# petuum/poseidon

Measured on AMD Instinct MI355X. Metric: images/sec (whole node), higher is better.
Workload: dtype bf16; 1 GPU; model=alexnet, global_batch=256, input=3x227x227, parallelism=dp1, sfb=False, hipgraph=True

## Files before the change

poseidon_amd/ops/csrc/bindings.cpp:

```cpp

#include <torch/extension.h>
#include <c10/hip/HIPStream.h>
#include <hip/hip_runtime.h>

#include <algorithm>
#include <atomic>
#include <cmath>
#include <cstdlib>
#include <utility>

#include "ps_api.h"
#include "ps_mt.h"

namespace {

using at::Tensor;

hipStream_t stream() { return c10::hip::getCurrentHIPStream().stream(); }

bool is_bf16(const Tensor& t) { return t.scalar_type() == at::kBFloat16; }

struct P {
  void* p;
  explicit P(const Tensor& t) : p(t.data_ptr()) {}
// ... 197 lines not shown
    const c10::optional<Tensor>& dw_acc,
    const c10::optional<Tensor>& dw_out) {
  check_float_like(dy, "dy");
  TORCH_CHECK(!(dw_acc.has_value() && dw_out.has_value()),
              "linear_backward: dw_acc and dw_out exclude each other");
  auto xc = x.contiguous();
  auto wc = linear_weight(w, w_shadow, is_bf16(dy));
  auto dyc = dy.contiguous();
  int M = xc.size(0), K = xc.size(1), N = wc.size(0);
  c10::optional<Tensor> dx, dw, db;
  if (need_dx) {
    Tensor t = at::empty({M, K}, x.options());
    run_gemm(dyc, wc, t, nullptr, M, K, N, N, K, K, 0, 0, 0, true, false,
             1.0f, 0.0f);
    dx = t;
  }
  if (need_dw) {
    const bool own = !dw_acc.has_value() && !dw_out.has_value();
    Tensor t = dw_acc.has_value() ? *dw_acc
               : dw_out.has_value()
                   ? *dw_out
                   : at::empty({N, K}, x.options().dtype(at::kFloat));
    TORCH_CHECK(t.is_cuda() && t.scalar_type() == at::kFloat &&
                t.is_contiguous() && t.dim() == 2 && t.size(0) == N &&
                t.size(1) == K,
                "linear_backward: dW target must be contiguous f32 [N,K]");
    run_gemm(dyc, xc, t, nullptr, N, K, M, N, K, K, 0, 0, 0, false, false,
             1.0f, dw_acc.has_value() ? 1.0f : 0.0f);
    if (own) dw = t;
  }
  if (has_bias) {
    Tensor t = at::zeros({N}, x.options().dtype(at::kFloat));
    colsum_into(dyc, t.data_ptr<float>(), M, N);
    db = t;
  }
  return {dx, dw, db};
}

Tensor gemm_at_b(const Tensor& a, const Tensor& b) {
  check_float_like(a, "a");
  auto ac = a.contiguous();
  auto bc = b.contiguous();
  int M = ac.size(0), N = ac.size(1), K = bc.size(1);
  Tensor t = at::empty({N, K}, a.options().dtype(at::kFloat));
  run_gemm(ac, bc, t, nullptr, N, K, M, N, K, K, 0, 0, 0, false, false,
           1.0f, 0.0f);
  return t;
}


enum { PS_PACKED_OFF = 0, PS_PACKED_ON = 1, PS_PACKED_AUTO = -1 };
enum { PS_ROWFUSED_OFF = 0, PS_ROWFUSED_ON = 1, PS_ROWFUSED_AUTO = -1 };

ConvPlan conv_plan_for(at::IntArrayRef x_shape, int Co, int kh, int kw,
                       int sh, int sw, int ph, int pw, int G, bool bf16,
                       int packed = PS_PACKED_AUTO,
                       int rowfused = PS_ROWFUSED_AUTO) {
  TORCH_CHECK(x_shape.size() == 4 && G > 0 && x_shape[1] % G == 0 &&
              Co % G == 0, "conv channel/group mismatch");
  const bool rf_auto = rowfused == PS_ROWFUSED_AUTO;
  const ConvPolicy policy = {
      g_implicit_gemm.load(), g_implicit_thresh.load(),
      g_dgrad_fwd_thresh.load(),
      packed == PS_PACKED_AUTO ? g_packed_conv.load() : packed == PS_PACKED_ON,
      rf_auto ? g_rowfused_conv.load() : rowfused == PS_ROWFUSED_ON,
      rf_auto ? g_rowfused_thresh.load() : 0,
      rf_auto && ps_deterministic() != 0};
  ConvPlan p = ps_conv_plan((int)x_shape[0], (int)x_shape[1], (int)x_shape[2],
                            (int)x_shape[3], Co, kh, kw, sh, sw, ph, pw, G,
                            bf16 ? 2 : 4, policy);
  if (p.rowfused && !ps_rowfused_prepare()) p.rowfused = false;
  return p;
}

py::dict conv_plan(std::vector<int64_t> x_shape, std::vector<int64_t> w_shape,
                   std::vector<int64_t> stride, std::vector<int64_t> pad,
                   int G, bool bf16) {
  TORCH_CHECK(w_shape.size() == 4 && stride.size() == 2 && pad.size() == 2);
  TORCH_CHECK(x_shape.size() == 4 && w_shape[1] * G == x_shape[1],
              "conv channel/group mismatch");
  const ConvPlan p = conv_plan_for(x_shape, (int)w_shape[0], (int)w_shape[2],
                                   (int)w_shape[3], (int)stride[0],
                                   (int)stride[1], (int)pad[0], (int)pad[1],
                                   G, bf16);
  py::dict d;
  d["N"] = p.g.N; d["C"] = p.g.C; d["H"] = p.g.H; d["W"] = p.g.W;
  d["Ho"] = p.g.Ho; d["Wo"] = p.g.Wo; d["G"] = p.g.G;
  d["Co"] = p.Co; d["Cg"] = p.Cg; d["Cog"] = p.Cog;
  d["Kg"] = p.Kg; d["Kcol"] = p.Kcol; d["NP"] = p.NP; d["vec"] = p.vec;
  d["is_1x1"] = p.is_1x1; d["ld_col"] = p.ld_col; d["wk_ld"] = p.wk_ld;
  d["kpad"] = p.kpad; d["implicit"] = p.implicit;
  d["Kgw_implicit"] = p.Kgw_implicit; d["dgrad_as_fwd"] = p.dgrad_as_fwd;
  d["packed"] = p.packed; d["pk_W"] = p.pk_W; d["pk_kw"] = p.pk_kw;
  d["pk_Kg"] = p.pk_Kg; d["kw_ld"] = p.kw_ld; d["c_ld"] = p.c_ld;
  d["rowfused"] = p.rowfused;
  d["Kgw"] = p.implicit ? p.Kgw_implicit : p.wk_ld;
  return d;
}

std::vector<int64_t> khwc_layout(int64_t Cg, int64_t kw, bool packed) {
  int kw_ld, c_ld;
  ps_khwc_layout((int)kw, (int)Cg, packed, &kw_ld, &c_ld);
  return {kw_ld, c_ld};
}

Tensor weight_khwc_tr(const Tensor& w, int G, bool bf16) {
// ... 10 lines not shown
std::vector<Tensor> conv2d_forward_ex(const Tensor& x, const Tensor& w,
                                      const c10::optional<Tensor>& bias,
                                      int sh, int sw, int ph, int pw, int G,
                                      bool fuse_relu,
                                      const c10::optional<Tensor>& wk_cached,
                                      const c10::optional<Tensor>& wkT_cached) {
  check_float_like(x, "x");
  const bool bf16 = is_bf16(x);
  TORCH_CHECK(x.dim() == 4 && w.size(1) * G == x.size(1),
              "conv channel/group mismatch");
  const ConvPlan p = conv_plan_for(x.sizes(), (int)w.size(0),
                                   (int)w.size(2), (int)w.size(3), sh, sw, ph,
                                   pw, G, bf16);
  const ConvGeom& g = p.g;
  const int Co = p.Co, Cog = p.Cog;
  Tensor x_cl = (p.is_1x1 || p.implicit) ? cl4(x) : Tensor();

  const auto cdt = bf16 ? at::kBFloat16 : at::kFloat;
  Tensor wk, wkT;
  if (wk_cached.has_value() && wkT_cached.has_value() &&
      wk_cached->scalar_type() == cdt) {
    TORCH_CHECK(wk_cached->size(1) == p.wk_ld, "conv2d_forward: cached wk is ",
                wk_cached->size(1), " wide, the plan's wk_ld is ", p.wk_ld);
    wk = *wk_cached;
    wkT = *wkT_cached;
  } else {
    auto wc = w.contiguous();
    auto wkopts = w.options().dtype(cdt);
    wk = p.kpad ? at::zeros({Co, (int64_t)p.wk_ld}, wkopts)
                : at::empty({Co, (int64_t)p.wk_ld}, wkopts);
    wkT = at::empty({(int64_t)p.Kcol, (int64_t)Cog}, wkopts);
    PS_CALL_W(weight_to_khwc_both, bf16, wc.data_ptr<float>(), P(wk), P(wkT),
            Co, p.Cg, g.kh, g.kw, G, p.wk_ld, p.kw_ld, p.c_ld, stream());
  }

  Tensor colT;
  if (p.rowfused) {
    TORCH_CHECK(x.numel() / g.N < (1LL << 31) &&
                (g.H - 1) * x.stride(2) + (g.W - 1) * x.stride(3) +
                (g.C - 1) * x.stride(1) < (1LL << 31),
                "row-fused conv: one image must span < 2^31 elements");
    TORCH_CHECK(wk.is_contiguous() && ((uintptr_t)wk.data_ptr() & 15) == 0,
                "row-fused conv: wk must be contiguous and 16 B aligned");
    const RowFusedTiling t = ps_rowfused_tiling(
        g.N, g.C, g.H, g.W, Co, g.kh, g.kw, g.sh, g.sw, g.ph, g.pw, p.wk_ld);
    Tensor y = empty_cl({g.N, Co, g.Ho, g.Wo}, x.options());
    Tensor bc;
    const float* bp = nullptr;
    if (bias.has_value()) {
      bc = bias->contiguous();
      bp = bc.data_ptr<float>();
    }
    ps_conv_rowfused_fwd(&t, x.data_ptr(), x.stride(0), x.stride(1),
                         x.stride(2), x.stride(3), wk.data_ptr(), bp,
                         y.data_ptr(), fuse_relu ? 1 : 0, stream());
    return {y, at::empty({0, (int64_t)p.ld_col}, x.options()), wkT};
  }
  if (p.packed) {
    colT = at::empty({g.N, g.H, (int64_t)p.pk_W, PS_PK_C}, x.options());
    ps_pack_pairs_bf16(x.data_ptr(), colT.data_ptr(), g.N, g.C, g.H, g.W,
                       p.pk_W, g.pw, x.stride(0), x.stride(1), x.stride(2),
                       x.stride(3), stream());
  } else if (p.is_1x1) {
    colT = rows2d(x_cl);
  } else if (!p.implicit) {
    colT = at::empty({p.NP, (int64_t)p.ld_col}, x.options());
    const bool staged = PS_CALL(im2col_rowstage, bf16, P(x), P(colT), &g,
                                p.ld_col, x.stride(0), x.stride(1),
                                x.stride(2), x.stride(3), stream());
    if (!staged) {
      const Tensor xc = cl4(x);
      PS_CALL(im2col_nhwc, bf16, P(xc), P(colT), &g, p.ld_col, stream());
      if (p.kpad)
        PS_CALL(zero_cols, bf16, P(colT), p.NP, p.ld_col, p.Kcol, stream());
    }
  }

  Tensor y = empty_cl({g.N, Co, g.Ho, g.Wo}, x.options());
  const float* bp = nullptr;
  Tensor bc;
  if (bias.has_value()) {
    bc = bias->contiguous();
    bp = bc.data_ptr<float>();
  }
  const int Kgl = p.wk_ld;
  const bool gather = p.implicit || p.packed;
  const Tensor& xg = p.packed ? colT : x_cl;
  for (int grp = 0; grp < G; ++grp) {
    GatherDesc ga{};
    if (gather)
      ga = ps_gather_desc(p, PS_GATHER_FWD, xg.data_ptr(), zero_page(xg), grp);
    run_gemm(gather ? xg : colT, wk, y, bp ? bp + grp * Cog : nullptr,
             (int)p.NP, Cog, Kgl,
             gather ? Kgl : p.ld_col, Kgl, Co,
             gather ? 0 : (int64_t)grp * Kgl,
             (int64_t)grp * Cog * Kgl,
             (int64_t)grp * Cog,
             true, true, 1.0f, 0.0f, gather ? &ga : nullptr, nullptr,
             fuse_relu);
  }
  if (!colT.defined())
    colT = at::empty({0}, x.options());
  return {y, colT, wkT};
}

Tensor conv2d_backward_input(const Tensor& w, const Tensor& dy,
                             std::vector<int64_t> x_shape, int sh, int sw,
                             int ph, int pw, int G,
// ... 38 lines not shown
  Tensor dcolT = p.is_1x1 ? rows2d(dx)
                          : at::empty({p.NP, (int64_t)p.Kcol}, dy.options());
  Tensor dy2 = rows2d(dy_cl);
  for (int grp = 0; grp < G; ++grp) {
    run_gemm(dy2, wkT, dcolT, nullptr,
             (int)p.NP, Kg, Cog,
             Co, Cog, p.Kcol,
             (int64_t)grp * Cog, (int64_t)grp * Kg * Cog,
             (int64_t)grp * Kg,
             true, true, 1.0f, 0.0f);
  }
  if (!p.is_1x1)
    PS_CALL(col2im_nhwc, bf16, P(dcolT), P(dx), &g, stream());
  return dx;
}

Tensor conv2d_backward_weight_acc(const Tensor& x, const Tensor& colT,
                                  const Tensor& dy, Tensor dw_out,
                                  c10::optional<Tensor> db_out,
                                  int sh, int sw, int ph, int pw, int G,
                                  const c10::optional<Tensor>& dwk_buf,
                                  bool skip_unpack, bool skip_db) {
  check_float_like(dy, "dy");
  auto dy_cl = cl4(dy);
  const bool implicit = colT.numel() == 0 && colT.dim() == 1;
  const bool packed = colT.dim() == 4;
  const bool rowfused = colT.dim() == 2 && colT.size(0) == 0;
  const ConvPlan p = conv_plan_for(x.sizes(), (int)dw_out.size(0),
                                   (int)dw_out.size(2), (int)dw_out.size(3),
                                   sh, sw, ph, pw, G, is_bf16(dy),
                                   packed ? PS_PACKED_ON : PS_PACKED_OFF,
                                   rowfused ? PS_ROWFUSED_ON : PS_ROWFUSED_OFF);
  TORCH_CHECK(dw_out.size(1) == p.Cg && dy_cl.size(2) == p.g.Ho &&
              dy_cl.size(3) == p.g.Wo, "conv wgrad: shape mismatch");
  const int Co = p.Co, Cog = p.Cog;
  if (rowfused) {
    TORCH_CHECK(p.rowfused && is_bf16(x) && is_bf16(dy),
                "conv wgrad: row-fused cache slot does not match the plan");
    TORCH_CHECK(!ps_deterministic(),
                "conv wgrad: the row-fused wgrad has no deterministic form");
    const ConvGeom& g = p.g;
    TORCH_CHECK(x.numel() / g.N < (1LL << 31) &&
                (g.H - 1) * x.stride(2) + (g.W - 1) * x.stride(3) +
                (g.C - 1) * x.stride(1) < (1LL << 31),
                "row-fused conv: one image must span < 2^31 elements");
    const int Kgw = p.wk_ld;
    const bool prez =
        dwk_buf.has_value() && dwk_buf->numel() == (int64_t)Co * Kgw;
    Tensor dwk = prez ? *dwk_buf
               : at::empty({Co, (int64_t)Kgw}, dy.options().dtype(at::kFloat));
    const RowFusedTiling t = ps_rowfused_tiling(
        g.N, g.C, g.H, g.W, Co, g.kh, g.kw, g.sh, g.sw, g.ph, g.pw, p.wk_ld);
    ps_conv_rowfused_wgrad(&t, x.data_ptr(), x.stride(0), x.stride(1),
                           x.stride(2), x.stride(3), dy_cl.data_ptr(),
                           dwk.data_ptr<float>(), prez ? 1 : 0, stream());
    if (!skip_unpack)
      ps_weight_from_khwc_f32(dwk.data_ptr<float>(), dw_out.data_ptr<float>(),
                              Co, p.Cg, g.kh, g.kw, Kgw,
                              1.0f, p.kw_ld, p.c_ld, stream());
    if (db_out.has_value() && !skip_db)
      colsum_into(dy_cl, db_out->data_ptr<float>(), p.NP, Co);
    return dwk;
  }
  if (packed) {
    TORCH_CHECK(p.packed && colT.is_contiguous() && is_bf16(colT) &&
                colT.size(0) == p.g.N && colT.size(1) == p.g.H &&
                colT.size(2) == p.pk_W && colT.size(3) == PS_PK_C,
                "conv wgrad: packed input does not match the plan");
  } else {
    TORCH_CHECK(implicit || colT.size(1) == p.ld_col,
                "conv wgrad: colT width does not match the plan");
  }
  const Tensor xg = packed ? colT : implicit ? cl4(x) : Tensor();
  const bool gather = implicit || packed;
  const int Kgw = implicit ? p.Kgw_implicit : p.wk_ld;

  const bool prez = dwk_buf.has_value() && dwk_buf->numel() == (int64_t)Co * Kgw;
  Tensor dwk = prez ? *dwk_buf
             : at::empty({Co, (int64_t)Kgw}, dy.options().dtype(at::kFloat));
  Tensor dy2 = rows2d(dy_cl);
  for (int grp = 0; grp < G; ++grp) {
    GatherDesc gb{};
    if (gather)
      gb = ps_gather_desc(p, PS_GATHER_WGRAD, xg.data_ptr(), zero_page(xg),
                          grp);
    run_gemm(dy2, gather ? xg : colT, dwk, nullptr,
             Cog, Kgw, (int)p.NP,
             Co, gather ? Kgw : p.ld_col, Kgw,
             (int64_t)grp * Cog,
             gather ? 0 : (int64_t)grp * Kgw,
             (int64_t)grp * Cog * Kgw,
             false, false, 1.0f, 0.0f, nullptr, gather ? &gb : nullptr,
             false, prez);
  }
  if (!skip_unpack)
    ps_weight_from_khwc_f32(dwk.data_ptr<float>(), dw_out.data_ptr<float>(),
                            Co, p.Cg, p.g.kh, p.g.kw, Kgw,
                            1.0f, p.kw_ld, p.c_ld, stream());
  if (db_out.has_value() && !skip_db)
    colsum_into(dy_cl, db_out->data_ptr<float>(), p.NP, Co);
  return dwk;
}


Tensor concat_channels(std::vector<Tensor> inputs) {
  TORCH_CHECK(!inputs.empty());
  auto x0 = cl4(inputs[0]);
  int64_t N = x0.size(0), H = x0.size(2), W = x0.size(3);
// ... 1025 lines not shown
```

poseidon_amd/ops/csrc/conv_rowfused.hip:

```cpp

#include "ps_common.h"
#include "ps_api.h"
#include "ps_rowfused.h"

#include <atomic>
#include <mutex>

namespace ps {
namespace {

constexpr int RF_THREADS = PS_RF_THREADS;
constexpr int RF_STAGERS = 256;

typedef __attribute__((ext_vector_type(4))) __bf16 rf_bf16x4;
typedef __attribute__((ext_vector_type(4))) int rf_i32x4;

struct RfX {
  const __bf16* x;
  int64_t sn;
  int sc, sh, sw;
};

__device__ inline __bf16 rf_read(const char* img, int pbase, int koff) {
  return *reinterpret_cast<const __bf16*>(img + max(pbase + koff, 0));
}

typedef __bf16 rf_uvec8 __attribute__((ext_vector_type(8), aligned(2)));

template <int NV, int NT>
__device__ inline void rf_load_x(bf16x8 (&xv)[NV], const RowFusedTiling& t,
                                 const RowFusedTile& tl, const RfX& X,
                                 int tid, int first) {
  const int vpr = t.rsw_ld / 8;
  const int total = t.srows * t.C * vpr;
  const int iw0 = tl.ow0 * t.sw - t.pw;
  const int ih0 = tl.oh0 * t.sh - t.ph;
  const __bf16* xn = X.x + tl.n * X.sn;
#pragma unroll
  for (int v = 0; v < NV; ++v) {
    const int idx = first + tid + v * NT;
    const int rc = idx / vpr;
    const int sr = rc / t.C;
    const int c = rc - sr * t.C;
    const int ih = ih0 + sr;
    const int iw = iw0 + (idx - rc * vpr) * 8;
#pragma unroll
    for (int j = 0; j < 8; ++j) xv[v][j] = (__bf16)0.0f;
    if (idx < total && ih >= 0 && ih < t.H) {
      const __bf16* src = xn + (ih * X.sh + c * X.sc);
      if (X.sw == 1 && iw >= 0 && iw + 8 <= t.W) {
        xv[v] = *reinterpret_cast<const rf_uvec8*>(src + iw);
      } else {
#pragma unroll
        for (int j = 0; j < 8; ++j)
          if (iw + j >= 0 && iw + j < t.W) xv[v][j] = src[(iw + j) * X.sw];
      }
    }
  }
}

template <int NV, int NT>
__device__ inline void rf_store_x(char* img, const bf16x8 (&xv)[NV],
                                  const RowFusedTiling& t, int tid,
                                  int first) {
  const int total = t.srows * t.C * (t.rsw_ld / 8);
#pragma unroll
  for (int v = 0; v < NV; ++v) {
    const int idx = first + tid + v * NT;
    if (idx < total)
      *reinterpret_cast<bf16x8*>(img + PS_RF_HDR + idx * 16) = xv[v];
  }
}

constexpr int RF_FV = 6;
__device__ inline void rf_stage_x(char* img, const RowFusedTiling& t,
                                  const RowFusedTile& tl, const RfX& X,
                                  int ptid) {
  const int total = t.srows * t.C * (t.rsw_ld / 8);
  for (int first = 0; first < total; first += RF_FV * RF_STAGERS) {
    bf16x8 xv[RF_FV];
    rf_load_x<RF_FV, RF_STAGERS>(xv, t, tl, X, ptid, first);
    rf_store_x<RF_FV, RF_STAGERS>(img, xv, t, ptid, first);
  }
}

__device__ inline void rf_zero_headers(char* xs0, int xs_bytes, int tid) {
  if (tid < 4) reinterpret_cast<int*>(xs0)[tid] = 0;
  else if (tid < 8) reinterpret_cast<int*>(xs0 + xs_bytes)[tid - 4] = 0;
}

template <int FN>
__global__ __launch_bounds__(RF_THREADS)
void conv_rowfused_fwd_k(RowFusedTiling t, RfX X,
                         const __bf16* __restrict__ wk,
                         const float* __restrict__ bias,
                         __bf16* __restrict__ y, int relu, float alpha,
                         int tpb) {
  extern __shared__ __attribute__((aligned(16))) char smem[];
  __bf16* wl = reinterpret_cast<__bf16*>(smem);
  int* kofft = reinterpret_cast<int*>(smem + t.fwd_koff_off);
  char* xs0 = smem + t.fwd_xs_off;
  const int tid = threadIdx.x;
  const int lane = tid & 63;
  const int wid = __builtin_amdgcn_readfirstlane(tid >> 6);
  const int l = lane & 15, q = lane >> 4;
  const int64_t t0 = (int64_t)blockIdx.x * tpb;
  const int64_t t1 = t0 + tpb < t.tiles ? t0 + tpb : t.tiles;
  if (t0 >= t1) return;

  {
    const int vpr = t.Kpad / 8;
    for (int i = tid; i < t.Cop * vpr; i += RF_THREADS) {
      const int co = i / vpr;
      const int kv = (i - co * vpr) * 8;
      bf16x8 v;
#pragma unroll
      for (int j = 0; j < 8; ++j) v[j] = (__bf16)0.0f;
      if (co < t.Co)
        v = *reinterpret_cast<const bf16x8*>(&wk[(int64_t)co * t.Kpad + kv]);
      *reinterpret_cast<bf16x8*>(&wl[co * t.w_ld + kv]) = v;
    }
    for (int k = tid; k < t.Kpad; k += RF_THREADS) kofft[k] = ps_rf_koff(t, k);
    rf_zero_headers(xs0, t.xs_bytes, tid);
  }
  if (wid >= 4)
    rf_stage_x(xs0, t, ps_rf_tile(t, t0), X, tid - RF_STAGERS);
  int pf[2], pbf[2];
#pragma unroll
  for (int f = 0; f < 2; ++f) {
    pf[f] = (wid & 3) * 32 + f * 16 + l;
    pbf[f] = ps_rf_pbase(t, pf[f]);
  }
  __syncthreads();

  for (int64_t ti = t0; ti < t1; ++ti) {
    const int cur = (int)(ti - t0) & 1;
    if (wid >= 4) {
      if (ti + 1 < t1)
        rf_stage_x(xs0 + (cur ^ 1) * t.xs_bytes, t, ps_rf_tile(t, ti + 1), X,
                   tid - RF_STAGERS);
    } else {
      const RowFusedTile tl = ps_rf_tile(t, ti);
      if (wid * 32 < tl.nlive) {
        const char* img = xs0 + cur * t.xs_bytes;
        int pb[2];
#pragma unroll
        for (int f = 0; f < 2; ++f)
          pb[f] = pf[f] < tl.nlive ? pbf[f] : PS_RF_NEG;
        f32x4 acc[2][FN] = {};
#pragma unroll 2
        for (int ks = 0; ks < t.Kpad; ks += 32) {
          const rf_i32x4 k0 =
              *reinterpret_cast<const rf_i32x4*>(&kofft[ks + q * 8]);
          const rf_i32x4 k1 =
              *reinterpret_cast<const rf_i32x4*>(&kofft[ks + q * 8 + 4]);
          bf16x8 bfr[FN];
#pragma unroll
          for (int fn = 0; fn < FN; ++fn)
            bfr[fn] = *reinterpret_cast<const bf16x8*>(
                &wl[(fn * 16 + l) * t.w_ld + ks + q * 8]);
          bf16x8 af[2];
#pragma unroll
          for (int f = 0; f < 2; ++f) {
#pragma unroll
            for (int e = 0; e < 4; ++e) {
              af[f][e] = rf_read(img, pb[f], k0[e]);
              af[f][4 + e] = rf_read(img, pb[f], k1[e]);
            }
          }
#pragma unroll
          for (int f = 0; f < 2; ++f)
#pragma unroll
            for (int fn = 0; fn < FN; ++fn)
              acc[f][fn] = __builtin_amdgcn_mfma_f32_16x16x32_bf16(
                  af[f], bfr[fn], acc[f][fn], 0, 0, 0);
        }
#pragma unroll
        for (int f = 0; f < 2; ++f) {
#pragma unroll
          for (int fn = 0; fn < FN; ++fn) {
            const int col = fn * 16 + l;
            if (col >= t.Co) continue;
            const float bv = bias ? bias[col] : 0.0f;
#pragma unroll
            for (int r = 0; r < 4; ++r) {
              const int p = wid * 32 + f * 16 + q * 4 + r;
              if (p >= tl.nlive) continue;
              float v = alpha * acc[f][fn][r] + bv;
              if (relu && v < 0.0f) v = 0.0f;
              from_f32(v, y[(tl.pos0 + p) * t.Co + col]);
            }
          }
        }
      }
    }
    __syncthreads();
  }
}

__device__ inline bf16x8 rf_tr_frag(unsigned base, int kk, int cb, int l,
                                    int ld) {
  const unsigned a1 =
      base + (unsigned)(((kk + (l >> 2)) * ld + cb + 4 * (l & 3)) * 2);
  const unsigned a2 = a1 + (unsigned)(4 * ld * 2);
  rf_bf16x4 v1, v2;
  asm volatile("ds_read_b64_tr_b16 %0, %2\n\t"
               "ds_read_b64_tr_b16 %1, %3"
               : "=&v"(v1), "=&v"(v2) : "v"(a1), "v"(a2));
  bf16x8 f;
#pragma unroll
  for (int i = 0; i < 4; ++i) { f[i] = v1[i]; f[4 + i] = v2[i]; }
  return f;
}

template <int N>
__device__ inline void rf_tr_wait(bf16x8 (&a)[N]) {
  asm volatile("s_waitcnt lgkmcnt(0)" ::: "memory");
#pragma unroll
  for (int i = 0; i < N; ++i) asm volatile("" : "+v"(a[i]));
}

template <int FN, int KF>
__global__ __launch_bounds__(RF_THREADS)
void conv_rowfused_wgrad_k(RowFusedTiling t, RfX X,
                           const __bf16* __restrict__ dy,
                           float* __restrict__ dwk, int tpb) {
  extern __shared__ __attribute__((aligned(16))) char smem[];
  int* ptab = reinterpret_cast<int*>(smem);
  __bf16* dyl0 = reinterpret_cast<__bf16*>(smem + t.wg_dy_off);
  char* xs0 = smem + t.wg_xs_off;
  const int dy_tile = PS_RF_TM * t.dy_ld;
  const int tid = threadIdx.x;
  const int lane = tid & 63;
  const int wid = __builtin_amdgcn_readfirstlane(tid >> 6);
  const int l = lane & 15, q = lane >> 4;
  const int64_t t0 = (int64_t)blockIdx.x * tpb;
  const int64_t t1 = t0 + tpb < t.tiles ? t0 + tpb : t.tiles;
  if (t0 >= t1) return;
  rf_zero_headers(xs0, t.xs_bytes, tid);

  const int my_pb = tid < PS_RF_TM ? ps_rf_pbase(t, tid) : 0;
  const int cv8 = t.Cop / 8;
  bf16x8 xv[PS_RF_XV], dv[PS_RF_DV];
  auto load = [&](int64_t ti) {
    const RowFusedTile tl = ps_rf_tile(t, ti);
    rf_load_x<PS_RF_XV, RF_THREADS>(xv, t, tl, X, tid, 0);
#pragma unroll
    for (int v = 0; v < PS_RF_DV; ++v) {
      const int idx = tid + v * RF_THREADS;
      const int p = idx / cv8;
      const int cv = (idx - p * cv8) * 8;
#pragma unroll
      for (int j = 0; j < 8; ++j) dv[v][j] = (__bf16)0.0f;
      if (p < tl.nlive && cv < t.Co)
        dv[v] = *reinterpret_cast<const bf16x8*>(
            &dy[(tl.pos0 + p) * t.Co + cv]);
    }
  };
  auto store = [&](int buf, int64_t ti) {
    const RowFusedTile tl = ps_rf_tile(t, ti);
    rf_store_x<PS_RF_XV, RF_THREADS>(xs0 + buf * t.xs_bytes, xv, t, tid,
                                     0);
    __bf16* dyl = dyl0 + buf * dy_tile;
#pragma unroll
    for (int v = 0; v < PS_RF_DV; ++v) {
      const int idx = tid + v * RF_THREADS;
      const int p = idx / cv8;
      const int cv = (idx - p * cv8) * 8;
      if (p < PS_RF_TM)
        *reinterpret_cast<bf16x8*>(&dyl[p * t.dy_ld + cv]) = dv[v];
    }
    if (tid < PS_RF_TM)
      ptab[buf * PS_RF_TM + tid] = tid < tl.nlive ? my_pb : PS_RF_NEG;
  };
  load(t0);
  store(0, t0);

  const int by = blockIdx.y;
  int kofs[KF];
  bool klive[KF];
#pragma unroll
  for (int i = 0; i < KF; ++i) {
    const int kf = (by * KF + i) * 8 + wid;
    klive[i] = kf * 16 < t.Kpad;
    kofs[i] = klive[i] ? ps_rf_koff(t, kf * 16 + l) : PS_RF_NEG;
  }
  f32x4 acc[FN][KF] = {};
  __syncthreads();

  for (int64_t ti = t0; ti < t1; ++ti) {
    const int cur = (int)(ti - t0) & 1;
    if (ti + 1 < t1) load(ti + 1);
    {
      const RowFusedTile tl = ps_rf_tile(t, ti);
      const char* img = xs0 + cur * t.xs_bytes;
      const int* pt = ptab + cur * PS_RF_TM;
      const unsigned dyb = (unsigned)(unsigned long long)(
          __attribute__((address_space(3))) __bf16*)(dyl0 + cur * dy_tile);
      for (int p0 = 0; p0 < tl.nlive; p0 += 32) {
        const rf_i32x4 pa =
            *reinterpret_cast<const rf_i32x4*>(&pt[p0 + q * 8]);
        const rf_i32x4 pb =
            *reinterpret_cast<const rf_i32x4*>(&pt[p0 + q * 8 + 4]);
        bf16x8 af[FN];
#pragma unroll
        for (int fn = 0; fn < FN; ++fn)
          af[fn] = rf_tr_frag(dyb, p0 + q * 8, fn * 16, l, t.dy_ld);
        rf_tr_wait(af);
#pragma unroll
        for (int i = 0; i < KF; ++i) {
          if (klive[i]) {
            bf16x8 bfr;
#pragma unroll
            for (int e = 0; e < 4; ++e) {
              bfr[e] = rf_read(img, pa[e], kofs[i]);
              bfr[4 + e] = rf_read(img, pb[e], kofs[i]);
            }
#pragma unroll
            for (int fn = 0; fn < FN; ++fn)
              acc[fn][i] = __builtin_amdgcn_mfma_f32_16x16x32_bf16(
                  af[fn], bfr, acc[fn][i], 0, 0, 0);
// ... 48 lines not shown
template <int FN>
void rf_launch_fwd(const RowFusedTiling& t, const RfX& X, const void* wk,
                   const float* bias, void* y, int relu, hipStream_t s) {
  int blocks, tpb;
  rf_grid(t, &blocks, &tpb);
  conv_rowfused_fwd_k<FN><<<dim3((unsigned)blocks), RF_THREADS, t.fwd_lds,
                            s>>>(t, X, (const __bf16*)wk, bias, (__bf16*)y,
                                 relu, 1.0f, tpb);
}

template <int FN, int KF>
void rf_launch_wgrad(const RowFusedTiling& t, const RfX& X, const void* dy,
                     float* dwk, hipStream_t s) {
  int blocks, tpb;
  rf_grid(t, &blocks, &tpb);
  const int gy = (t.Kpad / 16 + 8 * KF - 1) / (8 * KF);
  conv_rowfused_wgrad_k<FN, KF><<<dim3((unsigned)blocks, (unsigned)gy),
                                  RF_THREADS, t.wg_lds, s>>>(
      t, X, (const __bf16*)dy, dwk, tpb);
}

}
}

extern "C" {

void ps_rowfused_set_blocks(int n) { ps::g_rf_blocks.store(n < 0 ? 0 : n); }

int ps_rowfused_prepare() {
  using namespace ps;
  std::call_once(g_rf_once, [] {
    int dev = 0, n = 0;
    if (hipGetDevice(&dev) != hipSuccess ||
        hipDeviceGetAttribute(&n, hipDeviceAttributeMultiprocessorCount,
                              dev) != hipSuccess || n <= 0)
      return;
    const bool ok =
        rf_allow_lds(conv_rowfused_fwd_k<1>) &&
        rf_allow_lds(conv_rowfused_fwd_k<2>) &&
        rf_allow_lds(conv_rowfused_fwd_k<4>) &&
        rf_allow_lds(conv_rowfused_fwd_k<6>) &&
        rf_allow_lds(conv_rowfused_fwd_k<8>) &&
        rf_allow_lds(conv_rowfused_wgrad_k<1, 3>) &&
        rf_allow_lds(conv_rowfused_wgrad_k<2, 3>) &&
        rf_allow_lds(conv_rowfused_wgrad_k<4, 3>) &&
        rf_allow_lds(conv_rowfused_wgrad_k<6, 3>) &&
        rf_allow_lds(conv_rowfused_wgrad_k<8, 2>);
    if (ok) g_rf_cus.store(n);
  });
  return g_rf_cus.load() > 0 ? 1 : 0;
}

void ps_conv_rowfused_fwd(const RowFusedTiling* t, const void* x, int64_t sn,
                          int64_t sc, int64_t sh, int64_t sw, const void* wk,
                          const float* bias, void* y, int relu,
                          hipStream_t s) {
  const ps::RfX X = {(const __bf16*)x, sn, (int)sc, (int)sh, (int)sw};
  const int fn = t->Cop / 16;
  if (fn <= 1) ps::rf_launch_fwd<1>(*t, X, wk, bias, y, relu, s);
  else if (fn <= 2) ps::rf_launch_fwd<2>(*t, X, wk, bias, y, relu, s);
  else if (fn <= 4) ps::rf_launch_fwd<4>(*t, X, wk, bias, y, relu, s);
  else if (fn <= 6) ps::rf_launch_fwd<6>(*t, X, wk, bias, y, relu, s);
  else ps::rf_launch_fwd<8>(*t, X, wk, bias, y, relu, s);
}

void ps_conv_rowfused_wgrad(const RowFusedTiling* t, const void* x,
                            int64_t sn, int64_t sc, int64_t sh, int64_t sw,
                            const void* dy, float* dwk, int prezeroed,
                            hipStream_t s) {
  const ps::RfX X = {(const __bf16*)x, sn, (int)sc, (int)sh, (int)sw};
  if (!prezeroed)
    PS_HIP_CHECK(hipMemsetAsync(
        dwk, 0, (size_t)t->Co * t->Kpad * sizeof(float), s));
  ps_count_float_atomic();
  const int fn = t->Cop / 16;
  if (fn <= 1) ps::rf_launch_wgrad<1, 3>(*t, X, dy, dwk, s);
  else if (fn <= 2) ps::rf_launch_wgrad<2, 3>(*t, X, dy, dwk, s);
  else if (fn <= 4) ps::rf_launch_wgrad<4, 3>(*t, X, dy, dwk, s);
  else if (fn <= 6) ps::rf_launch_wgrad<6, 3>(*t, X, dy, dwk, s);
  else ps::rf_launch_wgrad<8, 2>(*t, X, dy, dwk, s);
}

}
```

poseidon_amd/ops/csrc/ps_api.h:

```cpp
#pragma once
#include <hip/hip_runtime.h>
#include <cstdint>

#include "ps_conv_plan.h"
#include "ps_gemm_plan.h"
#include "ps_stats_plan.h"
#include "ps_transform.h"

struct GemmArgs {
  const void* A;
  const void* B;
  void* C;
  const float* bias;
  int M, N, K;
  int64_t lda, ldb, ldc;
  float alpha, beta;
  bool a_klast, b_klast;
  bool in_bf16;
  bool out_f32;
  const GatherDesc* gather_a;
  const GatherDesc* gather_b;
  bool relu;
  bool c_prezeroed;
};
// ... 106 lines not shown
void ps_lrn_bwd_v8_tail_bf16(const void*, const void*, const void*,
                             const uint8_t*, const PoolGeom*, void*, float*,
                             int, int64_t, int, int, float, float, int,
                             hipStream_t);

void ps_softmax_rows_f32(const float*, float*, int64_t, int, hipStream_t);
void ps_softmax_bwd_rows_f32(const float*, const float*, float*, int64_t, int,
                             hipStream_t);
void ps_softmax_loss_fwd_f32(const float*, const float*, float*, float*,
                             float*, int64_t, int, hipStream_t);
void ps_softmax_loss_bwd_f32(const float*, const float*, float*, int64_t, int,
                             float, hipStream_t);
void ps_softmax_rows_bf16(const void*, void*, int64_t, int, hipStream_t);
void ps_softmax_bwd_rows_bf16(const void*, const void*, void*, int64_t, int,
                              hipStream_t);
void ps_softmax_loss_fwd_bf16(const void*, const float*, void*, float*,
                              float*, int64_t, int, hipStream_t);
void ps_softmax_loss_bwd_bf16(const void*, const float*, void*, int64_t, int,
                              float, hipStream_t);

void ps_sgd_update(float*, const float*, float*, int64_t, float, float, float,
                   hipStream_t);
void ps_nesterov_update(float*, const float*, float*, int64_t, float, float,
                        float, hipStream_t);
void ps_adagrad_update(float*, const float*, float*, int64_t, float, float,
                       float, hipStream_t);
void ps_f32_to_bf16(const float*, void*, int64_t, hipStream_t);
void ps_sgd_update_lrdev(float*, const float*, float*, int64_t, float, float,
                         float, const float*, hipStream_t);
void ps_u64_inc(void*, hipStream_t);
void ps_sgd_mt(const void* descs, const void* chunks, int nchunks, float lr,
               float mom, const float* lr_dev, hipStream_t);
void ps_zero_mt(const void* descs, const void* chunks, int nchunks,
                hipStream_t);
void ps_repack_mt(const void* descs, const void* chunks, int nchunks,
                  hipStream_t);
void ps_unpack_mt(const void* descs, const void* chunks, int nchunks,
                  hipStream_t);

void ps_blob_stats(const void* p, int64_t n, int bf16, int slot,
                   void* scratch, int* nblk, hipStream_t);
void ps_blob_stats_mt(const void* descs, const void* chunks, int nchunks,
                      void* scratch, int* nblk, hipStream_t);
void ps_blob_stats_finalize(const void* scratch, const int* nblk, void* stats,
                            int slot0, int nslots, hipStream_t);
int64_t ps_blob_stats_launches(int reset);

void ps_data_transform_f32(const uint8_t*, const int*, const float*, float*,
                           const TransformGeom*, hipStream_t);
void ps_data_transform_bf16(const uint8_t*, const int*, const float*, void*,
                            const TransformGeom*, hipStream_t);

void ps_conv_rowfused_fwd(const RowFusedTiling*, const void* x, int64_t sn,
                          int64_t sc, int64_t sh, int64_t sw, const void* wk,
                          const float* bias, void* y, int relu, hipStream_t);
void ps_conv_rowfused_wgrad(const RowFusedTiling*, const void* x, int64_t sn,
                            int64_t sc, int64_t sh, int64_t sw,
                            const void* dy, float* dwk, int prezeroed,
                            hipStream_t);
int ps_rowfused_prepare();
void ps_rowfused_set_blocks(int n);

void ps_chan_concat4_f32(float*, void* const*, const int*, int, int, int64_t,
                         int, int, const void* const*, hipStream_t);
void ps_chan_concat4_bf16(void*, void* const*, const int*, int, int, int64_t,
                          int, int, const void* const*, hipStream_t);
void ps_chan_copy_f32(const float*, float*, int64_t, int, int, int, hipStream_t);
void ps_chan_copy_bf16(const void*, void*, int64_t, int, int, int, hipStream_t);
void ps_chan_slice_f32(const float*, float*, int64_t, int, int, int, hipStream_t);
void ps_chan_slice_bf16(const void*, void*, int64_t, int, int, int, hipStream_t);
void ps_im2col_nhwc_f32(const float*, float*, const ConvGeom*, int ldcol,
                        hipStream_t);
bool ps_im2col_rowstage_f32(const float*, float*, const ConvGeom*, int ldcol,
                            int64_t sn, int64_t sc, int64_t sh, int64_t sw,
                            hipStream_t);
bool ps_im2col_rowstage_bf16(const void*, void*, const ConvGeom*, int ldcol,
                             int64_t sn, int64_t sc, int64_t sh, int64_t sw,
                             hipStream_t);
void ps_col2im_nhwc_f32(const float*, float*, const ConvGeom*, hipStream_t);
void ps_im2col_nhwc_bf16(const void*, void*, const ConvGeom*, int ldcol,
                         hipStream_t);
void ps_col2im_nhwc_bf16(const void*, void*, const ConvGeom*, hipStream_t);
void ps_weight_to_khwc_f32(const float*, float*, int, int, int, int, hipStream_t);
void ps_weight_to_khwc_f32_bf16(const float*, void*, int, int, int, int, hipStream_t);
void ps_zero_cols_f32(float*, int64_t rows, int ld, int c_lo, hipStream_t);
void ps_zero_cols_bf16(void*, int64_t rows, int ld, int c_lo, hipStream_t);
void ps_weight_to_dgrad_f32(const float*, float*, int, int, int, int, int,
                            hipStream_t);
void ps_weight_to_dgrad_f32_bf16(const float*, void*, int, int, int, int,
                                 int, hipStream_t);
void ps_weight_from_khwc_f32(const float*, float*, int, int, int, int,
                             int ld, float beta, int kw_ld, int c_ld,
                             hipStream_t);
void ps_weight_to_khwc_tr_f32(const float*, float*, int, int, int, int, int,
                              hipStream_t);
void ps_weight_to_khwc_tr_f32_bf16(const float*, void*, int, int, int, int,
                                   int, hipStream_t);
void ps_weight_to_khwc_both_f32(const float*, float*, float*, int, int, int,
                                int, int, int ldk, int kw_ld, int c_ld,
                                hipStream_t);
void ps_weight_to_khwc_both_f32_bf16(const float*, void*, void*, int, int,
                                     int, int, int, int ldk, int kw_ld,
                                     int c_ld, hipStream_t);
void ps_pack_pairs_bf16(const void* x, void* xp, int N, int C, int H, int W,
                        int Wp, int pw, int64_t sn, int64_t sc, int64_t sh,
                        int64_t sw, hipStream_t);
}
```

poseidon_amd/ops/csrc/ps_rowfused.h:

```cpp
#pragma once
#include <cstdint>

constexpr int PS_RF_TM = 128;
constexpr int PS_RF_THREADS = 512;
constexpr int PS_RF_XV = 3;
constexpr int PS_RF_DV = 4;
constexpr int PS_RF_MAX_CO = 128;
constexpr int PS_RF_LDS_MAX = 160 << 10;
constexpr int PS_RF_HDR = 16;
constexpr int PS_RF_WPAD = 8;
constexpr int PS_RF_DYPAD = 8;
constexpr int PS_RF_NEG = -(1 << 24);

struct RowFusedTiling {
  int C, H, W, Ho, Wo, kh, kw, sh, sw, ph, pw;
  int Co, Cop;
  int Kcol, Kpad;
  int RUN;
  int R, WS, segs;
  int row_tiles;
  int tiles_per_img;
  int64_t tiles;
  int srows;
  int rsw;
// ... 50 lines not shown
  const int64_t xs = PS_RF_HDR + (int64_t)t.srows * C * t.rsw_ld * 2;
  t.w_ld = Kpad + PS_RF_WPAD;
  t.dy_ld = t.Cop + PS_RF_DYPAD;
  const int64_t wbytes = (int64_t)t.Cop * t.w_ld * 2;
  const int64_t fwd = wbytes + (int64_t)Kpad * 4 + 2 * xs;
  const int64_t dyb = (int64_t)PS_RF_TM * t.dy_ld * 2;
  const int64_t wg = 2 * (int64_t)PS_RF_TM * 4 + 2 * dyb + 2 * xs;
  if (fwd > PS_RF_LDS_MAX || wg > PS_RF_LDS_MAX) return t;
  if ((int64_t)t.srows * C * (t.rsw_ld / 8) > PS_RF_THREADS * PS_RF_XV)
    return t;
  t.xs_bytes = (int)xs;
  t.fwd_koff_off = (int)wbytes;
  t.fwd_xs_off = (int)(wbytes + Kpad * 4);
  t.fwd_lds = (int)fwd;
  t.wg_dy_off = 2 * PS_RF_TM * 4;
  t.wg_xs_off = (int)(t.wg_dy_off + 2 * dyb);
  t.wg_lds = (int)wg;
  t.ok = true;
  return t;
}

#if defined(__HIPCC__)
#define PS_RF_HD __host__ __device__
#else
#define PS_RF_HD
#endif

PS_RF_HD inline RowFusedTile ps_rf_tile(const RowFusedTiling& t, int64_t ti) {
  RowFusedTile r;
  r.n = (int)(ti / t.tiles_per_img);
  const int rem = (int)(ti - (int64_t)r.n * t.tiles_per_img);
  const int strip = rem / t.segs;
  r.oh0 = strip * t.R;
  r.ow0 = (rem - strip * t.segs) * t.WS;
  const int rows = t.Ho - r.oh0 < t.R ? t.Ho - r.oh0 : t.R;
  const int cols = t.Wo - r.ow0 < t.WS ? t.Wo - r.ow0 : t.WS;
  r.nlive = t.segs == 1 ? rows * t.WS : cols;
  r.pos0 = ((int64_t)r.n * t.Ho + r.oh0) * t.Wo + r.ow0;
  return r;
}

PS_RF_HD inline int ps_rf_pbase(const RowFusedTiling& t, int p) {
  return PS_RF_HDR +
         ((p / t.WS) * t.sh * t.C * t.rsw_ld + (p % t.WS) * t.sw) * 2;
}
PS_RF_HD inline int ps_rf_koff(const RowFusedTiling& t, int k) {
  if (k >= t.Kcol) return PS_RF_NEG;
  return (((k / t.RUN) * t.C + k % t.C) * t.rsw_ld + (k % t.RUN) / t.C) * 2;
}
PS_RF_HD inline int ps_rf_addr(int pbase, int koff) {
  const int a = pbase + koff;
  return a < 0 ? 0 : a;
}
```

Before: 62730 images/sec.

## Widen row-fused conv input staging with span-bounded vector loads and masking

Reworks how the row-fused conv kernels stage input rows into LDS. A 16-byte load is now used whenever it stays inside the tensor's total span, and padding lanes are zeroed with a bitmask at store time, instead of falling back to per-element loads at image edges. Per-thread position math is hoisted out of the tile loop in wgrad. Bias values are preloaded into registers in the forward kernel, and an unroll pragma on the K loop is dropped. This adds a span argument to the API and more register state per thread, which may raise register pressure.

```diff
diff --git a/poseidon_amd/ops/csrc/bindings.cpp b/poseidon_amd/ops/csrc/bindings.cpp
--- a/poseidon_amd/ops/csrc/bindings.cpp
+++ b/poseidon_amd/ops/csrc/bindings.cpp
@@ -273,6 +273,16 @@
 enum { PS_PACKED_OFF = 0, PS_PACKED_ON = 1, PS_PACKED_AUTO = -1 };
 enum { PS_ROWFUSED_OFF = 0, PS_ROWFUSED_ON = 1, PS_ROWFUSED_AUTO = -1 };
 
+int64_t rowfused_span(const Tensor& x) {
+  int64_t span = 1;
+  for (int64_t d = 0; d < x.dim(); ++d) {
+    TORCH_CHECK(x.size(d) > 0 && x.stride(d) >= 0,
+                "row-fused conv: empty or negatively strided x");
+    span += (x.size(d) - 1) * x.stride(d);
+  }
+  return span;
+}
+
 ConvPlan conv_plan_for(at::IntArrayRef x_shape, int Co, int kh, int kw,
                        int sh, int sw, int ph, int pw, int G, bool bf16,
                        int packed = PS_PACKED_AUTO,
@@ -389,8 +399,9 @@
       bp = bc.data_ptr<float>();
     }
     ps_conv_rowfused_fwd(&t, x.data_ptr(), x.stride(0), x.stride(1),
-                         x.stride(2), x.stride(3), wk.data_ptr(), bp,
-                         y.data_ptr(), fuse_relu ? 1 : 0, stream());
+                         x.stride(2), x.stride(3), rowfused_span(x),
+                         wk.data_ptr(), bp, y.data_ptr(), fuse_relu ? 1 : 0,
+                         stream());
     return {y, at::empty({0, (int64_t)p.ld_col}, x.options()), wkT};
   }
   if (p.packed) {
@@ -535,8 +546,9 @@
     const RowFusedTiling t = ps_rowfused_tiling(
         g.N, g.C, g.H, g.W, Co, g.kh, g.kw, g.sh, g.sw, g.ph, g.pw, p.wk_ld);
     ps_conv_rowfused_wgrad(&t, x.data_ptr(), x.stride(0), x.stride(1),
-                           x.stride(2), x.stride(3), dy_cl.data_ptr(),
-                           dwk.data_ptr<float>(), prez ? 1 : 0, stream());
+                           x.stride(2), x.stride(3), rowfused_span(x),
+                           dy_cl.data_ptr(), dwk.data_ptr<float>(),
+                           prez ? 1 : 0, stream());
     if (!skip_unpack)
       ps_weight_from_khwc_f32(dwk.data_ptr<float>(), dw_out.data_ptr<float>(),
                               Co, p.Cg, g.kh, g.kw, Kgw,
diff --git a/poseidon_amd/ops/csrc/conv_rowfused.hip b/poseidon_amd/ops/csrc/conv_rowfused.hip
--- a/poseidon_amd/ops/csrc/conv_rowfused.hip
+++ b/poseidon_amd/ops/csrc/conv_rowfused.hip
@@ -17,58 +17,87 @@
 
 struct RfX {
   const __bf16* x;
-  int64_t sn;
-  int sc, sh, sw;
+  RowFusedX g;
 };
 
 __device__ inline __bf16 rf_read(const char* img, int pbase, int koff) {
   return *reinterpret_cast<const __bf16*>(img + max(pbase + koff, 0));
 }
 
-typedef __bf16 rf_uvec8 __attribute__((ext_vector_type(8), aligned(2)));
+typedef unsigned rf_u32x4a2 __attribute__((ext_vector_type(4), aligned(2)));
+typedef unsigned rf_u32x4 __attribute__((ext_vector_type(4)));
+
+struct RfRaw {
+  unsigned w[4];
+  unsigned e[8];
+  int m;
+};
+
+struct RfPos {
+  int rel, sc;
+};
 
 template <int NV, int NT>
-__device__ inline void rf_load_x(bf16x8 (&xv)[NV], const RowFusedTiling& t,
-                                 const RowFusedTile& tl, const RfX& X,
-                                 int tid, int first) {
-  const int vpr = t.rsw_ld / 8;
-  const int total = t.srows * t.C * vpr;
-  const int iw0 = tl.ow0 * t.sw - t.pw;
-  const int ih0 = tl.oh0 * t.sh - t.ph;
-  const __bf16* xn = X.x + tl.n * X.sn;
+__device__ inline void rf_positions(RfPos (&pos)[NV], const RowFusedTiling& t,
+                                    const RfX& X, int tid, int first) {
 #pragma unroll
   for (int v = 0; v < NV; ++v) {
-    const int idx = first + tid + v * NT;
-    const int rc = idx / vpr;
-    const int sr = rc / t.C;
-    const int c = rc - sr * t.C;
-    const int ih = ih0 + sr;
-    const int iw = iw0 + (idx - rc * vpr) * 8;
-#pragma unroll
-    for (int j = 0; j < 8; ++j) xv[v][j] = (__bf16)0.0f;
-    if (idx < total && ih >= 0 && ih < t.H) {
-      const __bf16* src = xn + (ih * X.sh + c * X.sc);
-      if (X.sw == 1 && iw >= 0 && iw + 8 <= t.W) {
-        xv[v] = *reinterpret_cast<const rf_uvec8*>(src + iw);
-      } else {
-#pragma unroll
-        for (int j = 0; j < 8; ++j)
-          if (iw + j >= 0 && iw + j < t.W) xv[v][j] = src[(iw + j) * X.sw];
-      }
+    const RowFusedVecPos p = ps_rf_vec_pos(t, X.g, first + tid + v * NT);
+    pos[v].rel = p.rel;
+    pos[v].sc = p.live ? p.sr << 16 | p.col : -1;
+  }
+}
+
+template <int NV>
+__device__ inline void rf_load_x(RfRaw (&xr)[NV], const RfPos (&pos)[NV],
+                                 const RowFusedTiling& t,
+                                 const RowFusedTile& tl, const RfX& X) {
+#pragma unroll
+  for (int v = 0; v < NV; ++v) {
+    const RowFusedVecPos p = {pos[v].sc >> 16, pos[v].sc & 0xffff, pos[v].rel,
+                              pos[v].sc >= 0};
+    const RowFusedVec d = ps_rf_vec_at(t, tl, X.g, p);
+    xr[v].m = d.kind | d.lo << 2 | d.hi << 6;
+#pragma unroll
+    for (int j = 0; j < 4; ++j) xr[v].w[j] = 0u;
+#pragma unroll
+    for (int j = 0; j < 8; ++j) xr[v].e[j] = (unsigned)xr[v].m;
+    if (d.kind == PS_RF_WIDE) {
+      const rf_u32x4a2 w = *reinterpret_cast<const rf_u32x4a2*>(X.x + d.off);
+#pragma unroll
+      for (int j = 0; j < 4; ++j) xr[v].w[j] = w[j];
+    }
+    if (d.kind == PS_RF_NARROW) {
+#pragma unroll
+      for (int j = 0; j < 8; ++j)
+        xr[v].e[j] = *reinterpret_cast<const unsigned short*>(
+            X.x + ps_rf_narrow_off(t, d, X.g.sw, j));
     }
   }
 }
 
 template <int NV, int NT>
-__device__ inline void rf_store_x(char* img, const bf16x8 (&xv)[NV],
+__device__ inline void rf_store_x(char* img, const RfRaw (&xr)[NV],
                                   const RowFusedTiling& t, int tid,
                                   int first) {
   const int total = t.srows * t.C * (t.rsw_ld / 8);
 #pragma unroll
   for (int v = 0; v < NV; ++v) {
     const int idx = first + tid + v * NT;
+    const int m = xr[v].m;
+    const bool narrow = (m & 3) == PS_RF_NARROW;
+    const unsigned em = ps_rf_elem_mask((m >> 2) & 15, m >> 6);
+    rf_u32x4 o;
+#pragma unroll
+    for (int i = 0; i < 4; ++i) {
+      const unsigned w = narrow ? xr[v].e[2 * i] | xr[v].e[2 * i + 1] << 16
+                                : xr[v].w[i];
+      const unsigned keep = ((em >> (2 * i) & 1u) ? 0x0000ffffu : 0u) |
+                            ((em >> (2 * i + 1) & 1u) ? 0xffff0000u : 0u);
+      o[i] = w & keep;
+    }
     if (idx < total)
-      *reinterpret_cast<bf16x8*>(img + PS_RF_HDR + idx * 16) = xv[v];
+      *reinterpret_cast<rf_u32x4*>(img + PS_RF_HDR + idx * 16) = o;
   }
 }
 
@@ -78,9 +107,11 @@
                                   int ptid) {
   const int total = t.srows * t.C * (t.rsw_ld / 8);
   for (int first = 0; first < total; first += RF_FV * RF_STAGERS) {
-    bf16x8 xv[RF_FV];
-    rf_load_x<RF_FV, RF_STAGERS>(xv, t, tl, X, ptid, first);
-    rf_store_x<RF_FV, RF_STAGERS>(img, xv, t, ptid, first);
+    RfPos pos[RF_FV];
+    RfRaw xr[RF_FV];
+    rf_positions<RF_FV, RF_STAGERS>(pos, t, X, ptid, first);
+    rf_load_x<RF_FV>(xr, pos, t, tl, X);
+    rf_store_x<RF_FV, RF_STAGERS>(img, xr, t, ptid, first);
   }
 }
 
@@ -131,6 +162,12 @@
     pf[f] = (wid & 3) * 32 + f * 16 + l;
     pbf[f] = ps_rf_pbase(t, pf[f]);
   }
+  float bvf[FN];
+#pragma unroll
+  for (int fn = 0; fn < FN; ++fn)
+    bvf[fn] = bias && fn * 16 + l < t.Co ? bias[fn * 16 + l] : 0.0f;
+#pragma unroll
+  for (int fn = 0; fn < FN; ++fn) asm volatile("" : "+v"(bvf[fn]));
   __syncthreads();
 
   for (int64_t ti = t0; ti < t1; ++ti) {
@@ -148,7 +185,6 @@
         for (int f = 0; f < 2; ++f)
           pb[f] = pf[f] < tl.nlive ? pbf[f] : PS_RF_NEG;
         f32x4 acc[2][FN] = {};
-#pragma unroll 2
         for (int ks = 0; ks < t.Kpad; ks += 32) {
           const rf_i32x4 k0 =
               *reinterpret_cast<const rf_i32x4*>(&kofft[ks + q * 8]);
@@ -181,7 +217,7 @@
           for (int fn = 0; fn < FN; ++fn) {
             const int col = fn * 16 + l;
             if (col >= t.Co) continue;
-            const float bv = bias ? bias[col] : 0.0f;
+            const float bv = bvf[fn];
 #pragma unroll
             for (int r = 0; r < 4; ++r) {
               const int p = wid * 32 + f * 16 + q * 4 + r;
@@ -241,15 +277,24 @@
 
   const int my_pb = tid < PS_RF_TM ? ps_rf_pbase(t, tid) : 0;
   const int cv8 = t.Cop / 8;
-  bf16x8 xv[PS_RF_XV], dv[PS_RF_DV];
+  RfPos xpos[PS_RF_XV];
+  rf_positions<PS_RF_XV, RF_THREADS>(xpos, t, X, tid, 0);
+  int dyp[PS_RF_DV], dyc[PS_RF_DV];
+#pragma unroll
+  for (int v = 0; v < PS_RF_DV; ++v) {
+    const int idx = tid + v * RF_THREADS;
+    dyp[v] = idx / cv8;
+    dyc[v] = (idx - dyp[v] * cv8) * 8;
+  }
+  RfRaw xr[PS_RF_XV];
+  bf16x8 dv[PS_RF_DV];
   auto load = [&](int64_t ti) {
     const RowFusedTile tl = ps_rf_tile(t, ti);
-    rf_load_x<PS_RF_XV, RF_THREADS>(xv, t, tl, X, tid, 0);
+    rf_load_x<PS_RF_XV>(xr, xpos, t, tl, X);
 #pragma unroll
     for (int v = 0; v < PS_RF_DV; ++v) {
-      const int idx = tid + v * RF_THREADS;
-      const int p = idx / cv8;
-      const int cv = (idx - p * cv8) * 8;
+      const int p = dyp[v];
+      const int cv = dyc[v];
 #pragma unroll
       for (int j = 0; j < 8; ++j) dv[v][j] = (__bf16)0.0f;
       if (p < tl.nlive && cv < t.Co)
@@ -259,14 +304,13 @@
   };
   auto store = [&](int buf, int64_t ti) {
     const RowFusedTile tl = ps_rf_tile(t, ti);
-    rf_store_x<PS_RF_XV, RF_THREADS>(xs0 + buf * t.xs_bytes, xv, t, tid,
+    rf_store_x<PS_RF_XV, RF_THREADS>(xs0 + buf * t.xs_bytes, xr, t, tid,
                                      0);
     __bf16* dyl = dyl0 + buf * dy_tile;
 #pragma unroll
     for (int v = 0; v < PS_RF_DV; ++v) {
-      const int idx = tid + v * RF_THREADS;
-      const int p = idx / cv8;
-      const int cv = (idx - p * cv8) * 8;
+      const int p = dyp[v];
+      const int cv = dyc[v];
       if (p < PS_RF_TM)
         *reinterpret_cast<bf16x8*>(&dyl[p * t.dy_ld + cv]) = dv[v];
     }
@@ -421,10 +465,11 @@
 }
 
 void ps_conv_rowfused_fwd(const RowFusedTiling* t, const void* x, int64_t sn,
-                          int64_t sc, int64_t sh, int64_t sw, const void* wk,
-                          const float* bias, void* y, int relu,
-                          hipStream_t s) {
-  const ps::RfX X = {(const __bf16*)x, sn, (int)sc, (int)sh, (int)sw};
+                          int64_t sc, int64_t sh, int64_t sw, int64_t span,
+                          const void* wk, const float* bias, void* y,
+                          int relu, hipStream_t s) {
+  const ps::RfX X = {(const __bf16*)x,
+                     {sn, (int)sc, (int)sh, (int)sw, span}};
   const int fn = t->Cop / 16;
   if (fn <= 1) ps::rf_launch_fwd<1>(*t, X, wk, bias, y, relu, s);
   else if (fn <= 2) ps::rf_launch_fwd<2>(*t, X, wk, bias, y, relu, s);
@@ -435,9 +480,10 @@
 
 void ps_conv_rowfused_wgrad(const RowFusedTiling* t, const void* x,
                             int64_t sn, int64_t sc, int64_t sh, int64_t sw,
-                            const void* dy, float* dwk, int prezeroed,
-                            hipStream_t s) {
-  const ps::RfX X = {(const __bf16*)x, sn, (int)sc, (int)sh, (int)sw};
+                            int64_t span, const void* dy, float* dwk,
+                            int prezeroed, hipStream_t s) {
+  const ps::RfX X = {(const __bf16*)x,
+                     {sn, (int)sc, (int)sh, (int)sw, span}};
   if (!prezeroed)
     PS_HIP_CHECK(hipMemsetAsync(
         dwk, 0, (size_t)t->Co * t->Kpad * sizeof(float), s));
diff --git a/poseidon_amd/ops/csrc/ps_api.h b/poseidon_amd/ops/csrc/ps_api.h
--- a/poseidon_amd/ops/csrc/ps_api.h
+++ b/poseidon_amd/ops/csrc/ps_api.h
@@ -182,10 +182,11 @@
                             const TransformGeom*, hipStream_t);
 
 void ps_conv_rowfused_fwd(const RowFusedTiling*, const void* x, int64_t sn,
-                          int64_t sc, int64_t sh, int64_t sw, const void* wk,
-                          const float* bias, void* y, int relu, hipStream_t);
+                          int64_t sc, int64_t sh, int64_t sw, int64_t span,
+                          const void* wk, const float* bias, void* y,
+                          int relu, hipStream_t);
 void ps_conv_rowfused_wgrad(const RowFusedTiling*, const void* x, int64_t sn,
-                            int64_t sc, int64_t sh, int64_t sw,
+                            int64_t sc, int64_t sh, int64_t sw, int64_t span,
                             const void* dy, float* dwk, int prezeroed,
                             hipStream_t);
 int ps_rowfused_prepare();
diff --git a/poseidon_amd/ops/csrc/ps_rowfused.h b/poseidon_amd/ops/csrc/ps_rowfused.h
--- a/poseidon_amd/ops/csrc/ps_rowfused.h
+++ b/poseidon_amd/ops/csrc/ps_rowfused.h
@@ -126,3 +126,82 @@
   const int a = pbase + koff;
   return a < 0 ? 0 : a;
 }
+
+struct RowFusedX {
+  int64_t sn;
+  int sc, sh, sw;
+  int64_t span;
+};
+
+enum { PS_RF_ZERO = 0, PS_RF_WIDE = 1, PS_RF_NARROW = 2 };
+
+struct RowFusedVec {
+  int kind;
+  int lo, hi;
+  int iw;
+  int64_t off;
+};
+
+struct RowFusedVecPos {
+  int sr;
+  int col;
+  int rel;
+  bool live;
+};
+
+PS_RF_HD inline RowFusedVecPos ps_rf_vec_pos(const RowFusedTiling& t,
+                                             const RowFusedX& X, int idx) {
+  RowFusedVecPos p;
+  const int vpr = t.rsw_ld / 8;
+  const int rc = idx / vpr;
+  p.sr = rc / t.C;
+  p.col = (idx - rc * vpr) * 8;
+  p.rel = p.sr * X.sh + (rc - p.sr * t.C) * X.sc;
+  p.live = idx < t.srows * t.C * vpr;
+  return p;
+}
+
+PS_RF_HD inline RowFusedVec ps_rf_vec_at(const RowFusedTiling& t,
+                                         const RowFusedTile& tl,
+                                         const RowFusedX& X,
+                                         const RowFusedVecPos& p) {
+  RowFusedVec d;
+  const int ih0 = tl.oh0 * t.sh - t.ph;
+  const int ih = ih0 + p.sr;
+  d.iw = tl.ow0 * t.sw - t.pw + p.col;
+  d.lo = d.iw < 0 ? (d.iw < -8 ? 8 : -d.iw) : 0;
+  d.hi = t.W - d.iw < 8 ? (t.W - d.iw < 0 ? 0 : t.W - d.iw) : 8;
+  d.kind = PS_RF_ZERO;
+  d.off = 0;
+  if (!p.live || ih < 0 || ih >= t.H || d.lo >= d.hi) {
+    d.lo = d.hi = 0;
+    return d;
+  }
+  const int64_t row = tl.n * X.sn + (ih0 * X.sh + p.rel);
+  const int64_t first = row + d.iw;
+  if (X.sw == 1 && first >= 0 && first + 8 <= X.span) {
+    d.kind = PS_RF_WIDE;
+    d.off = first;
+  } else {
+    d.kind = PS_RF_NARROW;
+    d.off = row;
+  }
+  return d;
+}
+
+PS_RF_HD inline RowFusedVec ps_rf_vec(const RowFusedTiling& t,
+                                      const RowFusedTile& tl,
+                                      const RowFusedX& X, int idx) {
+  return ps_rf_vec_at(t, tl, X, ps_rf_vec_pos(t, X, idx));
+}
+
+PS_RF_HD inline int64_t ps_rf_narrow_off(const RowFusedTiling& t,
+                                         const RowFusedVec& d, int sw, int j) {
+  int px = d.iw + j;
+  px = px < 0 ? 0 : px > t.W - 1 ? t.W - 1 : px;
+  return d.off + (int64_t)px * sw;
+}
+
+PS_RF_HD inline unsigned ps_rf_elem_mask(int lo, int hi) {
+  return ((1u << hi) - 1u) & ~((1u << lo) - 1u);
+}
```

Measured after the change: 66030 images/sec (median of 6 runs). 5.3% higher.
